# CederGroupHub/smol

Measured on AMD Instinct MI355X. Metric: attempted MC flips/s (node) + ns/flip/replica, 4096-site FCC canonical, higher is better.
Workload: dtype f64

## Files before the change

### smol_amd/codeobj.py

```python

import hashlib
import os
import shutil
import struct
import subprocess

_MAGIC = b"__CLANG_OFFLOAD_BUNDLE__"
_CACHE = {}


def _code_objects(blob):
    pos = blob.find(_MAGIC)
    while pos >= 0:
        (n,) = struct.unpack_from("<Q", blob, pos + len(_MAGIC))
        q = pos + len(_MAGIC) + 8
        for _ in range(n):
            off, size, tlen = struct.unpack_from("<QQQ", blob, q)
            triple = blob[q + 24:q + 24 + tlen].decode()
            q += 24 + tlen
            if triple.startswith("hip") and "amdgcn" in triple and size:
                yield blob[pos + off:pos + off + size]
        pos = blob.find(_MAGIC, pos + len(_MAGIC))


def _elf_symbols(elf):
    if elf[:4] != b"\x7fELF" or elf[4] != 2:
        return [], None
    shoff, = struct.unpack_from("<Q", elf, 0x28)
    shentsize, shnum, _ = struct.unpack_from("<HHH", elf, 0x3A)
    sec = [struct.unpack_from("<IIQQQQIIQQ", elf, shoff + i * shentsize) for i in range(shnum)]
    syms = []
    for s in sec:
        if s[1] != 2:
            continue
        stroff = sec[s[6]][4]
        for k in range(s[5] // 24):
            nm, info, _, shndx, value, size = struct.unpack_from("<IBBHQQ", elf, s[4] + 24 * k)
            end = elf.index(b"\0", stroff + nm)
            syms.append((elf[stroff + nm:end].decode(), info & 0xF, shndx, value, size))

    def read(shndx, value, size):
        s = sec[shndx]
        if s[1] == 8:
            return b""
        o = s[4] + (value - s[3])
        return elf[o:o + size]

    return syms, read


def _demangle(names):
    exe = shutil.which("c++filt") or shutil.which("llvm-cxxfilt") or "/opt/rocm/lib/llvm/bin/llvm-cxxfilt"
    if not (exe and os.path.exists(exe)):
        return list(names)
    out = subprocess.run([exe], input="\n".join(names), capture_output=True, text=True, check=True).stdout
    dem = out.split("\n")[:len(names)]
    return dem if len(dem) == len(names) else list(names)


def _merge_copies(copies):
    return {n: (next(iter(c)) if len(c) == 1 else hashlib.sha256("".join(sorted(c)).encode()).hexdigest())
            for n, c in copies.items()}


def kernel_digests(path=None):
    if path is None:
        from . import engine
        path = os.environ.get("SMOLMC_LIB") or engine.LIB_PATH
    st = os.stat(path)
    key = (os.path.abspath(path), st.st_mtime_ns, st.st_size)
    if key in _CACHE:
        return _CACHE[key]
    with open(path, "rb") as fh:
        blob = fh.read()
    copies = {}
    for elf in _code_objects(blob):
        syms, read = _elf_symbols(elf)
        if read is None:
            continue
        kd = {n[:-3]: (sh, v, sz) for n, t, sh, v, sz in syms if n.endswith(".kd") and 0 < sh < 0xFF00}
        for n, t, sh, v, sz in syms:
            if t != 2 or n not in kd or not (0 < sh < 0xFF00):
                continue
            h = hashlib.sha256()
            h.update(read(sh, v, sz))
            h.update(read(*kd[n]))
            copies.setdefault(n, set()).add(h.hexdigest())
    raw = _merge_copies(copies)
    names = sorted(raw)
    out = {d: raw[m] for m, d in zip(names, _demangle(names))}
    _CACHE[key] = out
    return out


def _norm(name):
    return name.replace(" ", "")


def find_kernel(fragment, path=None):
    f = _norm(fragment)
    hits = [(n, d) for n, d in kernel_digests(path).items() if f in _norm(n)]
    return hits[0] if len(hits) == 1 else None


def isa_stale(entry, path=None):
    if not entry:
        return False
    if entry.get("isa_sha256") and entry.get("kernel_symbol"):
        hit = find_kernel(entry["kernel_symbol"], path)
        return hit is None or hit[1] != entry["isa_sha256"]
    from . import engine
    return entry.get("csrc_sha256") != engine.source_digest()


if __name__ == "__main__":
    import sys

    for name, dig in sorted(kernel_digests(sys.argv[1] if len(sys.argv) > 1 else None).items()):
        print(dig[:16], name[:160])
```

### smol_amd/csrc/mc_lean.h

```cpp
#pragma once
#include "smolmc_common.h"

template <int CTRL> __device__ __forceinline__ double dpp_xor_add(double v) {
    const int lo = __builtin_amdgcn_update_dpp(__double2loint(v), __double2loint(v), CTRL, 0xf, 0xf, true);
    const int hi = __builtin_amdgcn_update_dpp(__double2hiint(v), __double2hiint(v), CTRL, 0xf, 0xf, true);
    return v + __hiloint2double(hi, lo);
}
__device__ __forceinline__ double wave_sum_all(double v) {
    v = dpp_xor_add<0xB1>(v);
    v = dpp_xor_add<0x4E>(v);
    v = dpp_xor_add<0x141>(v);
    v = dpp_xor_add<0x140>(v);
    {
        const unsigned lo = (unsigned)__double2loint(v), hi = (unsigned)__double2hiint(v);
        const auto a = __builtin_amdgcn_permlane16_swap(lo, lo, false, false);
        const auto b = __builtin_amdgcn_permlane16_swap(hi, hi, false, false);
        v = __hiloint2double((int)b[0], (int)a[0]) + __hiloint2double((int)b[1], (int)a[1]);
    }
    {
        const unsigned lo = (unsigned)__double2loint(v), hi = (unsigned)__double2hiint(v);
        const auto a = __builtin_amdgcn_permlane32_swap(lo, lo, false, false);
        const auto b = __builtin_amdgcn_permlane32_swap(hi, hi, false, false);
        v = __hiloint2double((int)b[0], (int)a[0]) + __hiloint2double((int)b[1], (int)a[1]);
    }
    return v;
}

template <int CTRL> __device__ __forceinline__ float dpp_add_f32(float v) {
    const int t = __builtin_amdgcn_update_dpp(0, __float_as_int(v), CTRL, 0xf, 0xf, true);
    return v + __int_as_float(t);
}
__device__ __forceinline__ float wave_sum_f32_uniform(float v) {
    v = dpp_add_f32<0xB1>(v);
    v = dpp_add_f32<0x4E>(v);
    v = dpp_add_f32<0x141>(v);
    v = dpp_add_f32<0x140>(v);
    float total;
    asm volatile("s_nop 1\n\t"
                 "v_add_f32_dpp %1, %1, %1 row_bcast:15 row_mask:0xa bank_mask:0xf\n\t"
                 "s_nop 1\n\t"
                 "v_add_f32_dpp %1, %1, %1 row_bcast:31 row_mask:0xc bank_mask:0xf\n\t"
                 "s_nop 1\n\t"
                 "v_readlane_b32 %0, %1, 63\n\t"
                 "s_nop 1"
                 : "=s"(total), "+v"(v));
    return total;
}

typedef double smolmc_v4d __attribute__((ext_vector_type(4)));
__device__ __forceinline__ double wave_sum_mfma(double v) {
    const smolmc_v4d z = {0.0, 0.0, 0.0, 0.0};
    const smolmc_v4d d = __builtin_amdgcn_mfma_f64_16x16x4f64(v, 1.0, z, 0, 0, 0);
    const double t = (d[0] + d[1]) + (d[2] + d[3]);
    const smolmc_v4d d2 = __builtin_amdgcn_mfma_f64_16x16x4f64(t, 1.0, z, 0, 0, 0);
    return d2[0];
}
#ifdef SMOLMC_MFMA_REDUCE
#define LEAN_WAVE_SUM wave_sum_mfma
#else
#define LEAN_WAVE_SUM wave_sum_all
#endif

__device__ __forceinline__ double lean_ewald_partial(const LeanParams &P, const uint8_t *occ, int lane,
                                                     int s, int swa, int swm, int swb) {
    const double *g = P.ew_G + (size_t)s * P.ew_nact;
    const int W = P.ew_W, na = P.ew_nact;
    double out = 0;
    for (int j0 = lane; j0 < na; j0 += 64 * 8) {
        int k[8];
        double gk[8], q[8];
#pragma unroll
        for (int u = 0; u < 8; ++u) {
            const int jj = min(j0 + 64 * u, na - 1);
            k[u] = P.ew_act[jj];
            gk[u] = g[jj];
        }
#pragma unroll
        for (int u = 0; u < 8; ++u)
            q[u] = P.ew_qs[(size_t)k[u] * W + (int)occ[lean_swz(k[u], swa, swm, swb)]];
#pragma unroll
        for (int u = 0; u < 8; ++u)
            out = fma((j0 + 64 * u < na && k[u] != s) ? q[u] : 0.0, gk[u], out);
    }
    return out;
}

template <int FOOT = 2, bool PRE = false>
__device__ __forceinline__ void field_apply(const LeanParams &P, double *phi, int lane, int s, double dq,
                                            const uint32_t (&e0)[27], const bool have_e0) {
    const int js = s - P.sbase;
    const double keep = phi[js];
    const LeanParamsKernarg Q = rare_params();
    const unsigned char *gx = (const unsigned char *)Q->ew_gx;
    if (gx != nullptr) {
        const uint32_t *E8 = Q->ew_E8;
        const uint32_t s8[1] = {Q->ew_S8[js]};
        const double d[1] = {dq};
        if (PRE && have_e0) field_sweep_gx_pre27(phi, E8, gx, lane, P.ew_nact, s8, d, e0);
        else field_sweep_gx_multi<1, FOOT>(phi, E8, gx, lane, P.ew_nact, s8, d);
    } else {
        const double *g = P.ew_G + (size_t)s * P.ew_nact;
        field_sweep<false>(phi, g, g, lane, P.ew_nact, dq, 0.0);
    }
    phi[js] = keep;
}

template <int FOOT = 2>
__device__ __forceinline__ void field_apply(const LeanParams &P, double *phi, int lane, int s, double dq) {
    const uint32_t none[27] = {};
    field_apply<FOOT, false>(P, phi, lane, s, dq, none, false);
}

template <int FOOT = 1, bool FEW = false>
__device__ __forceinline__ void field_apply_flips(double *phi, int lane, int nfl, int vsite, double vdq) {
    const LeanParamsKernarg Q = rare_params();

    const unsigned char *gx = (const unsigned char *)Q->ew_gx;
    auto site_of = [&](int f) { return (int)rdlane((uint32_t)vsite, f); };
    auto dq_of = [&](int f) {
        return __hiloint2double((int)rdlane((uint32_t)__double2hiint(vdq), f), (int)rdlane((uint32_t)__double2loint(vdq), f));
    };
    const int sb = Q->sbase, na = Q->ew_nact;
    if (gx == nullptr) {
        const double *G = Q->ew_G;
        for (int f = 0; f < nfl; ++f) {
            const double dqf = dq_of(f);
            if (dqf == 0.0) continue;
            const double *g = G + (size_t)site_of(f) * na;
            field_sweep<false>(phi, g, g, lane, na, dqf, 0.0);
        }
        return;
    }
    const uint32_t *E8 = Q->ew_E8, *S8 = Q->ew_S8;
    for (int f0 = 0; f0 < nfl; f0 += 4) {
        const int n = min(4, nfl - f0);
        uint32_t s8[4];
        double dq[4];
#pragma unroll
        for (int k = 0; k < 4; ++k) {
            const int f = k < n ? f0 + k : f0;
            s8[k] = S8[site_of(f) - sb];
            dq[k] = k < n ? dq_of(f) : 0.0;
        }
        if (FEW && n <= 3) {
            const uint32_t a[3] = {s8[0], s8[1], s8[2]};
            const double d[3] = {dq[0], dq[1], dq[2]};
            field_sweep_gx_multi<3, FOOT>(phi, E8, gx, lane, na, a, d);
        } else if (n == 1) {
            const uint32_t a[1] = {s8[0]};
            const double d[1] = {dq[0]};
            field_sweep_gx_multi<1, FOOT>(phi, E8, gx, lane, na, a, d);
        } else if (n == 2) {
            const uint32_t a[2] = {s8[0], s8[1]};
            const double d[2] = {dq[0], dq[1]};
            field_sweep_gx_multi<2, FOOT>(phi, E8, gx, lane, na, a, d);
        } else if (n == 3) {
            const uint32_t a[3] = {s8[0], s8[1], s8[2]};
            const double d[3] = {dq[0], dq[1], dq[2]};
            field_sweep_gx_multi<3, FOOT>(phi, E8, gx, lane, na, a, d);
        } else {
            field_sweep_gx_multi<4, FOOT>(phi, E8, gx, lane, na, s8, dq);
        }
    }
}

template <int FOOT = 1>
__device__ __forceinline__ void field_apply2(const LeanParams &P, double *phi, int lane, int s1, double dq1,
                                             int s2, double dq2) {
    const int j1 = s1 - P.sbase, j2 = s2 - P.sbase;
    const LeanParamsKernarg Q = rare_params();
    const unsigned char *gx = (const unsigned char *)Q->ew_gx;
    if (gx != nullptr) {
        const uint32_t *E8 = Q->ew_E8, *S8 = Q->ew_S8;
        const uint32_t s8[2] = {S8[j1], S8[j2]};
        const double d[2] = {dq1, dq2};
        field_sweep_gx_multi<2, FOOT>(phi, E8, gx, lane, P.ew_nact, s8, d);
        return;
    }
    const double *g1 = P.ew_G + (size_t)s1 * P.ew_nact, *g2 = P.ew_G + (size_t)s2 * P.ew_nact;
    const double keep1 = phi[j1], keep2 = phi[j2];
    const double c12 = g2[j1], c21 = g1[j2];
    field_sweep<true>(phi, g1, g2, lane, P.ew_nact, dq1, dq2);
    if (j1 != j2) {
        phi[j1] = fma(dq2, c12, keep1);
        phi[j2] = fma(dq1, c21, keep2);
    } else {
        phi[j1] = keep1;
    }
}

__device__ __forceinline__ uint32_t bounded(uint32_t a, uint32_t lim) {
#ifdef SMOLMC_BOUNDS
    if (a >= lim) __builtin_trap();
#else
    (void)lim;
#endif
    return a;
}

template <int NW> struct RowWords { uint32_t w[NW]; };
template <int NW>
__device__ __forceinline__ RowWords<NW> load_row(__amdgpu_buffer_rsrc_t rs, uint32_t voff, uint32_t soff) {
    RowWords<NW> r;
    if constexpr (NW == 2) {
        const auto v = __builtin_amdgcn_raw_buffer_load_b64(rs, voff, soff, 0);
        r.w[0] = v[0]; r.w[1] = v[1];
    } else if constexpr (NW == 3) {
        const auto v = __builtin_amdgcn_raw_buffer_load_b96(rs, voff, soff, 0);
        r.w[0] = v[0]; r.w[1] = v[1]; r.w[2] = v[2];
    } else if constexpr (NW == 4) {
        const auto v = __builtin_amdgcn_raw_buffer_load_b128(rs, voff, soff, 0);
        r.w[0] = v[0]; r.w[1] = v[1]; r.w[2] = v[2]; r.w[3] = v[3];
    } else if constexpr (NW == 6) {
        const auto v = __builtin_amdgcn_raw_buffer_load_b128(rs, voff, soff, 0);
        const auto u = __builtin_amdgcn_raw_buffer_load_b64(rs, voff + 16u, soff, 0);
        r.w[0] = v[0]; r.w[1] = v[1]; r.w[2] = v[2]; r.w[3] = v[3]; r.w[4] = u[0]; r.w[5] = u[1];
    } else {
        static_assert(NW % 4 == 0, "row width");
#pragma unroll
        for (int b = 0; b < NW / 4; ++b) {
            const auto v = __builtin_amdgcn_raw_buffer_load_b128(rs, voff + 16u * b, soff, 0);
            r.w[4 * b] = v[0]; r.w[4 * b + 1] = v[1]; r.w[4 * b + 2] = v[2]; r.w[4 * b + 3] = v[3];
        }
    }
    return r;
}
template <int NW> __device__ __forceinline__ uint32_t row_entry(const RowWords<NW> &r, int q) {
    return (r.w[q >> 1] >> (16 * (q & 1))) & 0xffffu;
}
template <bool WIDE, int NW> __device__ __forceinline__ uint32_t row_addr(const RowWords<NW> &r, int q) {
    if constexpr (WIDE) return r.w[q];
    else return row_entry<NW>(r, q);
}

__device__ __noinline__ double wl_flatness_check(const double *wl_S, long long *wl_Hh, int L, double flat,
                                                 double div, double wl_m, int lane) {
    long cnt = 0;
    double sum = 0;
    for (int i = lane; i < L; i += 64)
        if (wl_S[i] > 0) { cnt++; sum += (double)wl_Hh[i]; }
    const double tcnt = wave_sum_all((double)cnt), tsum = wave_sum_all(sum);
    if (tcnt >= 2.0) {
        const double thr = flat * (tsum / tcnt);
        int bad = 0;
        for (int i = lane; i < L; i += 64)
            if (wl_S[i] > 0 && !((double)wl_Hh[i] > thr)) bad = 1;
        if (__ballot(bad) == 0ull) {
            for (int i = lane; i < L; i += 64) wl_Hh[i] = 0;
            wl_m = wl_m / div;
        }
    }
    return wl_m;
}

__device__ __noinline__ double wl_multi_flatness_check(const double *S, uint32_t *cnt, double *occb, long long *hist_g,
                                                       long long *occ_g, int L, double flat, double div, double wl_m, int lane) {
    long n = 0;
    double sum = 0;
    for (int i = lane; i < L; i += 64)
        if (S[i] > 0) { n++; sum += (double)(hist_g[i] + (long long)cnt[i]); }
    const double tn = wave_sum_all((double)n), tsum = wave_sum_all(sum);
    if (tn >= 2.0) {
        const double thr = flat * (tsum / tn);
        int bad = 0;
        for (int i = lane; i < L; i += 64)
            if (S[i] > 0 && !((double)(hist_g[i] + (long long)cnt[i]) > thr)) bad = 1;
        if (__ballot(bad) == 0ull) {
            for (int i = lane; i < L; i += 64) {
                hist_g[i] = 0;
                occ_g[i] += (long long)cnt[i];
                if (occb) occb[i] += (double)cnt[i];
                cnt[i] = 0u;
            }
            wl_m = wl_m / div;
        }
    }
    return wl_m;
}

typedef __attribute__((address_space(3))) uint8_t lds_u8_t;
typedef __attribute__((address_space(3))) double lds_f64_t;
#if defined(__HIP_DEVICE_COMPILE__)
#define SMOLMC_LDS_U8(a) (*(lds_u8_t *)(a))
#define SMOLMC_LDS_F64(a) (*(const lds_f64_t *)(a))
#define SMOLMC_LDS_F32(a) (*(const __attribute__((address_space(3))) float *)(a))
#else
#define SMOLMC_LDS_F32(a) (*(const float *)(uintptr_t)(a))
#define SMOLMC_LDS_U8(a) (*(uint8_t *)(uintptr_t)(a))
#define SMOLMC_LDS_F64(a) (*(const double *)(uintptr_t)(a))
#endif
template <bool ABS> __device__ __forceinline__ uint8_t occ_ld(const uint8_t *occ, uint32_t a) {
    if constexpr (ABS) return SMOLMC_LDS_U8(a);
    else return occ[a];
}
__device__ __forceinline__ uint32_t opaque_u32(uint32_t v) {
    asm volatile("" : "+s"(v));
    return v;
}
template <bool ABS> __device__ __forceinline__ void occ_st(uint8_t *occ, uint32_t a, uint8_t v) {
    if constexpr (ABS) SMOLMC_LDS_U8(a) = v;
    else occ[a] = v;
}

template <int NSLOT, int MM, int STEP, bool HAS_MU, int EWM, bool WL, bool BIAS = false, bool SOLO = false,
          int KF = 0, int OCC = 0, bool REPLAY = false>
__global__ void __attribute__((amdgpu_waves_per_eu(OCC ? OCC : 1, OCC ? OCC : 8)))
__launch_bounds__(256) mc_lean_kernel(const LeanParams P) {
    static_assert(KF == 0 || (!WL && !BIAS && !SOLO), "correlation-function tables: plain Metropolis layouts only");
    static_assert(!REPLAY || (!WL && OCC == 0), "replay: Metropolis variants (Wang-Landau: mc_wl_kernel)");
    constexpr int NACC = KF ? KF : 1;
    constexpr bool HAS_EW = EWM != 0, ew_field = EWM == 2;
    extern __shared__ __attribute__((aligned(16))) unsigned char smem[];
    if ((uint32_t)(uintptr_t)smem != 0u) __builtin_trap();
    const int lane = threadIdx.x & 63;
    const int wave = SOLO ? 0 : threadIdx.x >> 6;
    const int nwaves = SOLO ? 1 : blockDim.x >> 6;
    const int r = uni(blockIdx.x * nwaves + wave);
    const size_t per_wave = (size_t)P.Nlds + 64 * 8 + (WL ? (size_t)P.wl.L * 24 : 0) +
                            ((HAS_EW && ew_field) ? 64 + (size_t)P.ew_nact * 8 : 0);
    double *s_dt = SOLO ? (double *)(smem + ((per_wave + 15) & ~(size_t)15)) : (double *)smem;
    const uint32_t dt_off = SOLO ? (uint32_t)((per_wave + 15) & ~(size_t)15) : 0u;
    double *s_mu = s_dt + P.dt_len;
    double *s_q = s_mu + 8, *s_dg = s_mu + 16;
    unsigned char *wbase = SOLO ? smem : (unsigned char *)(s_mu + 24) + (size_t)wave * per_wave;
    uint8_t *occ = wbase;
    double *s_feat = (double *)(wbase + P.Nlds);
    double *wl_S = s_feat + 64;
    long long *wl_Hh = (long long *)(wl_S + (WL ? P.wl.L : 0));
    long long *wl_Oc = wl_Hh + (WL ? P.wl.L : 0);
    double *phi = (double *)(wbase + P.Nlds + 64 * 8 + 64);
    const int swa = P.swz_a, swm = P.swz_m, swb = P.swz_b;
    for (int i = threadIdx.x; i < P.dt_len; i += blockDim.x) s_dt[i] = P.dt[i];
#ifdef SMOLMC_EXP_F32TAB
    constexpr bool F32TAB = SOLO && STEP == SMOLMC_STEP_SWAP && !HAS_EW && !WL && !BIAS && KF == 0 && !REPLAY;
    const uint32_t sh_off = dt_off + (uint32_t)(P.dt_len + 24) * 8u;
    if (F32TAB) {
        float *s_dt32 = (float *)(smem + sh_off);
        for (int i = threadIdx.x; i < P.dt_len; i += blockDim.x) s_dt32[i] = (float)P.dt[i];
    }
#else
    constexpr bool F32TAB = false;
#endif
    if (HAS_MU && threadIdx.x < 8) s_mu[threadIdx.x] = threadIdx.x < P.ncodes ? P.mu_row[threadIdx.x] : 0.0;
    if (HAS_EW && ew_field && threadIdx.x < 8) {
        s_q[threadIdx.x] = P.ew_qrow[threadIdx.x];
        s_dg[threadIdx.x] = P.ew_dgrow[threadIdx.x];
    }
    const bool live = r < P.R;
    if (live) {
        const uint32_t *src = (const uint32_t *)(P.occ + (size_t)r * P.Npad);
        for (int i = lane; i < P.Npad / 4; i += 64)
            *(uint32_t *)(occ + lean_swz(4 * i, swa, swm, swb)) = src[i];
        s_feat[lane] = (WL && lane < P.F) ? P.features[(size_t)r * P.F + lane] : 0.0;
        if (HAS_EW && ew_field)
            for (int j = lane; j < P.ew_nact; j += 64) phi[j] = P.ew_phi[(size_t)r * P.ew_nact + j];
        if (WL)
            for (int i = lane; i < P.wl.L; i += 64) {
                wl_S[i] = P.wl.entropy[(size_t)r * P.wl.L + i];
                wl_Hh[i] = P.wl.hist[(size_t)r * P.wl.L + i];
                wl_Oc[i] = P.wl.occur[(size_t)r * P.wl.L + i];
            }
    }
    __syncthreads();
    if (!live) return;

#ifdef SMOLMC_NO_EWALD_E8REG
    constexpr bool EPRE = false;
#else
    constexpr bool EPRE = HAS_EW && STEP == SMOLMC_STEP_FLIP && !REPLAY;
#endif
    uint32_t ereg[27] = {};
    bool epre_on = false;
    if (EPRE) {
        const LeanParamsKernarg Q = rare_params();
        const uint32_t *E8 = Q->ew_E8;
        epre_on = ew_field && Q->ew_gx != nullptr && (Q->ew_nact >> 6) >= 27;
        if (epre_on) {
#pragma unroll
            for (int u = 0; u < 27; ++u) ereg[u] = E8[64 * u + lane];
        }
    }

    uint32_t doff8[NSLOT], st8[NSLOT][MM], sfeat[NSLOT];
    double wgt[NSLOT], acc[NSLOT], sfs[NSLOT];
    double accK[NSLOT][NACC];
    uint32_t kslot[NSLOT];
#pragma unroll
    for (int it = 0; it < NSLOT; ++it) {
        const LeanSlot sl = P.slots[it * 64 + lane];
        doff8[it] = sl.doff8 + dt_off;
        sfeat[it] = sl.feat;
        sfs[it] = sl.live ? sl.fs : 0.0;
        kslot[it] = sl.live;
#pragma unroll
        for (int m = 0; m < MM; ++m) st8[it][m] = sl.stride8[m];
        wgt[it] = sl.w;
        acc[it] = 0.0;
#pragma unroll
        for (int k = 0; k < NACC; ++k) accK[it][k] = 0.0;
    }
    const int wl_stride = WL ? P.F : 64;
    const int wl_k = WL ? max(1, min(8, 63 / max(wl_stride, 1))) : 1;
    uint32_t sfeat_wl[NSLOT];
#pragma unroll
    for (int it = 0; it < NSLOT; ++it) sfeat_wl[it] = sfeat[it] + (uint32_t)((lane % wl_k) * wl_stride);
    int wl_rd[8];
#pragma unroll
    for (int k = 0; k < 8; ++k) wl_rd[k] = (WL && k < wl_k && lane < wl_stride) ? lane + k * wl_stride : 63;
    auto wl_cur_feat = [&]() -> double {
        const int f = lane < wl_stride ? lane : 0;
        double t[8];
#pragma unroll
        for (int k = 0; k < 8; ++k) t[k] = k < wl_k ? s_feat[f + (k < wl_k ? k : 0) * wl_stride] : 0.0;
        return ((t[0] + t[1]) + (t[2] + t[3])) + ((t[4] + t[5]) + (t[6] + t[7]));
    };
    auto reduce_features = [&](double *dst) {
#pragma unroll
        for (int it = 0; it < NSLOT; ++it) {
            if (KF == 0) {
                __hip_atomic_fetch_add(&dst[sfeat[it]], sfs[it] * acc[it], __ATOMIC_RELAXED,
                                       __HIP_MEMORY_SCOPE_WAVEFRONT);
            } else {
#pragma unroll
                for (int k = 0; k < NACC; ++k) {
                    const bool on = (uint32_t)k < kslot[it];
                    __hip_atomic_fetch_add(&dst[sfeat[it] + (on ? k : 0)], on ? sfs[it] * accK[it][k] : 0.0,
                                           __ATOMIC_RELAXED, __HIP_MEMORY_SCOPE_WAVEFRONT);
                }
            }
        }
    };
#ifdef SMOLMC_EXP_CLOCK
    const long long ck0 = clock64(), wk0 = wall_clock64();
#endif
    double H = P.enthalpy[r];
    const double nbeta = WL ? 0.0 : -P.beta[r];
    double wl_m = WL ? P.wl.m[r] : 0.0;
    double wl_bq = WL ? floordiv_exact(H - P.wl.vmin, P.wl.bin) : 0.0;
    const double wl_inv_bin = WL ? 1.0 / P.wl.bin : 0.0;
    long long wl_counter = WL ? P.wl.counter[r] : 0;
    long long wl_rem_check = WL ? (P.wl.check ? wl_counter % P.wl.check : 1) : 0;
    unsigned long long step = P.nsteps[r];
    uint32_t nacc_add = 0;
    const uint32_t key0 = (uint32_t)P.seeds[r], key1 = (uint32_t)(P.seeds[r] >> 32);
    const uint32_t nact = (uint32_t)P.nact, nt8 = P.nt8, snt8 = P.snt8;
    const int sbase = P.sbase;
    double acc_mu = 0.0, acc_ew = 0.0;
    const int btype = BIAS ? P.bias_type : 0;
    const int brows = (btype && btype != SMOLMC_BIAS_FUGACITY) ? P.bias_rows : 0;
    double bias_acc = 0.0, chg[SMOLMC_MAX_BIAS_ROWS];
#pragma unroll
    for (int k = 0; k < SMOLMC_MAX_BIAS_ROWS; ++k) chg[k] = k < brows ? P.charge[(size_t)r * SMOLMC_MAX_BIAS_ROWS + k] : 0.0;
    constexpr bool FAST = !WL && !HAS_EW;
    float thr_lo = 0.0f, thr_hi = 0.0f;
    const double inv_nbeta = FAST ? 1.0 / nbeta : 0.0;
    uint32_t nacc_before = 0;
    int nsite = 0, naddr = 0;
    double *featp = P.features + (size_t)r * P.F;
    const double base_feat = lane < P.F ? featp[lane] : 0.0;
    uint32_t smp_countdown = P.smp.every ? (uint32_t)P.smp.every : 0xffffffffu;
    long long smp_index = 0;
    uint32_t W0 = 0;
    int cand[4] = {0, 0, 0, 0}, canda[4] = {0, 0, 0, 0};
    double vGc = 0.0;
    double logu = 0.0;
    unsigned long long batch64_base = ~0ull;
    unsigned long long batch_base = ~0ull;
    constexpr int ROW = NSLOT * MM;
    constexpr int NW = SOLO ? ROW : ROW / 2;
    constexpr uint32_t ENT = SOLO ? 4u : 2u;
    constexpr uint32_t SITE_BYTES = 64u * ROW * ENT;
    const __amdgpu_buffer_rsrc_t idx_rs = __builtin_amdgcn_make_buffer_rsrc(
        SOLO ? (void *)P.idx32 : (void *)P.idx, 0, 0x7fffffff, 0x00020000);
    const uint32_t lane_voff = (uint32_t)lane * (ROW * ENT);

    int s1, a1;
    RowWords<NW> row1;
    uint32_t ridx = 0;
    double lu_rp = 0.0;
    int rp_bad = 0;
    auto rp_site = [&](const uint32_t i) -> int {
        const int v = uni(P.rp_steps[((size_t)r * (uint32_t)P.steps + i) * 4]);
        return v >= 0 ? v : sbase;
    };
    {
        if (REPLAY) {
            s1 = rp_site(0u);
        } else {
            const unsigned long long sp = step - 1ull;
            const uint32_t w = (uint32_t)uni((int)philox4x32_10((uint32_t)sp, (uint32_t)(sp >> 32), 0u, 0u,
                                                                key0, key1).w[1]);
            s1 = sbase + (int)__umulhi(w, nact);
        }
        a1 = lean_swz(s1, swa, swm, swb);
        row1 = load_row<NW>(idx_rs, lane_voff, (uint32_t)s1 * SITE_BYTES);
    }

    double *wl_pend = WL ? P.wl.meanf + (size_t)r * P.wl.L * P.F : nullptr;
    double wl_pc[8] = {0.0, 0.0, 0.0, 0.0, 0.0, 0.0, 0.0, 0.0};
    auto wl_pend_sum = [&]() -> double {
        return ((wl_pc[0] + wl_pc[1]) + (wl_pc[2] + wl_pc[3])) + ((wl_pc[4] + wl_pc[5]) + (wl_pc[6] + wl_pc[7]));
    };
#ifdef SMOLMC_EXP_PHASES
    long long lph[5] = {0, 0, 0, 0, 0};
    long long lph_t = clock64();
#endif
    uint32_t steps_left = (uint32_t)P.steps;
    while (steps_left != 0u) {
        const unsigned long long base = step & ~15ull;
        if (!REPLAY && base != batch_base) {
            batch_base = base;
            const unsigned long long st = base + (unsigned)(lane >> 2);
            const philox_out o = philox4x32_10((uint32_t)st, (uint32_t)(st >> 32), (uint32_t)(lane & 3),
                                               0u, key0, key1);
            W0 = o.w[0];
            nsite = sbase + (int)__umulhi(o.w[1], nact);
            naddr = lean_swz(nsite, swa, swm, swb);
            if ((step & ~63ull) != batch64_base) {
                batch64_base = step & ~63ull;
                const unsigned long long s64 = batch64_base + (unsigned)lane;
                const philox_out a = philox4x32_10((uint32_t)s64, (uint32_t)(s64 >> 32), 0u, 0u, key0, key1);
                logu = log(philox_u53(a.w[2], a.w[3]));
                if (FAST) {
                    const double thr = logu * inv_nbeta;
                    const double eps = (F32TAB ? 2.0 : 1.0) * P.fast_eps + 1e-6 * fabs(thr);
                    thr_lo = P.fast_eps > 0.0 ? (float)(thr - eps) : -INFINITY;
                    thr_hi = P.fast_eps > 0.0 ? (float)(thr + eps) : INFINITY;
                }
            }
            if (STEP == SMOLMC_STEP_SWAP) {
                cand[0] = sbase + (int)__umulhi(o.w[0], nact);
                cand[1] = sbase + (int)__umulhi(o.w[1], nact);
                cand[2] = sbase + (int)__umulhi(o.w[2], nact);
                cand[3] = sbase + (int)__umulhi(o.w[3], nact);
#pragma unroll
                for (int j = 0; j < 4; ++j) canda[j] = lean_swz(cand[j], swa, swm, swb);
                if (HAS_EW && ew_field) {
                    const int prev = __shfl(nsite, (lane & ~3) - 4);
                    const int site_l = lane < 4 ? s1 : prev;
                    vGc = P.ew_G[(size_t)cand[0] * P.ew_nact + (site_l - sbase)];
                }
            }
        }
        uint32_t chunk = 16u - (uint32_t)(step & 15ull);
        chunk = min(chunk, steps_left);
        chunk = min(chunk, smp_countdown);
        steps_left -= chunk;
        smp_countdown -= chunk;
        const unsigned long long chunk_end = step + chunk;
        int l4 = (int)(step & 15ull) * 4;
        int l64 = (int)(step & 63ull);
        do {
#ifndef SMOLMC_NO_SETPRIO
        __builtin_amdgcn_s_setprio(1);
#endif
#ifdef SMOLMC_EXP_PHASES
        { const long long tn = clock64(); lph[0] += tn - lph_t; lph_t = tn; }
#endif
        int s1n, a1n;
        int rq1 = 0, rq2 = -1, rq3 = 0;
        bool rp_empty = false;
        if (REPLAY) {
            const int *rec = P.rp_steps + ((size_t)r * (uint32_t)P.steps + ridx) * 4;
            const int q0 = uni(rec[0]);
            rq1 = uni(rec[1]); rq2 = uni(rec[2]); rq3 = uni(rec[3]);
            rp_empty = q0 < 0;
            double u = uni_d(P.rp_u[(size_t)r * (uint32_t)P.steps + ridx]);
            if (u != u) u = 0.0;
            lu_rp = log(u);
            s1n = ridx + 1u < (uint32_t)P.steps ? rp_site(ridx + 1u) : s1;
            a1n = lean_swz(s1n, swa, swm, swb);
            if (FAST) {
                const double thr = lu_rp * inv_nbeta, eps = P.fast_eps + 1e-6 * fabs(thr);
                thr_lo = P.fast_eps > 0.0 ? (float)(thr - eps) : -INFINITY;
                thr_hi = P.fast_eps > 0.0 ? (float)(thr + eps) : INFINITY;
            }
        } else {
            s1n = (int)rdlane((uint32_t)nsite, l4);
            a1n = (int)rdlane((uint32_t)naddr, l4);
        }
        uint32_t va1 = (uint32_t)a1;
        asm volatile("" : "+v"(va1));
        const int o1 = uni((int)occ_ld<SOLO>(occ, va1));
        int nfl, s2, a2, n1, n2 = 0, o2 = 0;
        if (STEP != SMOLMC_STEP_SWAP) { s2 = s1; a2 = a1; }
        int fb = -1;
        if (REPLAY) {
            if (STEP == SMOLMC_STEP_FLIP) {
                nfl = rp_empty ? 0 : 1;
                n1 = rp_empty ? o1 : rq1;
                rp_bad |= (rq2 >= 0) ? 1 : 0;
            } else if (!rp_empty && rq2 >= 0) {
                nfl = 2;
                s2 = rq2;
                a2 = lean_swz(s2, swa, swm, swb);
                o2 = uni((int)occ_ld<SOLO>(occ, (uint32_t)a2));
                n2 = rq3;
                n1 = rq1;
                rp_bad |= (n2 != o1 || n1 != o2) ? 1 : 0;
                n2 = o1; n1 = o2;
            } else {
                nfl = 0; s2 = s1; a2 = a1; o2 = o1; n2 = o1; n1 = o1;
                rp_bad |= (!rp_empty || rq2 >= 0) ? 1 : 0;
            }
        } else if (STEP == SMOLMC_STEP_FLIP) {
            const uint32_t kk = __umulhi(rdlane(W0, l4 + 1), (uint32_t)(P.ncodes - 1));
            n1 = (int)kk + ((int)kk >= o1 ? 1 : 0);
            nfl = 1;
        } else {
            nfl = 2;
            n2 = o1;
#define SMOLMC_CAND_MASK(J)                                                                        \
    const int v##J = (int)occ_ld<SOLO>(occ, (uint32_t)canda[J]);                                   \
    const unsigned long long m##J = __ballot(v##J != o1) & (0xEull << l4);
#define SMOLMC_CAND_TAKE(J)                                                                        \
    {                                                                                              \
        const int b = __ffsll((long long)m##J) - 1;                                                \
        s2 = (int)rdlane((uint32_t)cand[J], b);                                                    \
        a2 = (int)rdlane((uint32_t)canda[J], b);                                                   \
        o2 = (int)rdlane((uint32_t)v##J, b);                                                       \
        if (J == 0) fb = b;                                                                        \
    }
            SMOLMC_CAND_MASK(0)
            if (m0) SMOLMC_CAND_TAKE(0)
            else {
                SMOLMC_CAND_MASK(1)
                if (m1) SMOLMC_CAND_TAKE(1)
                else {
                    SMOLMC_CAND_MASK(2)
                    if (m2) SMOLMC_CAND_TAKE(2)
                    else {
                        SMOLMC_CAND_MASK(3)
                        if (m3) SMOLMC_CAND_TAKE(3)
                        else {
                            bool hit = false;
                            const unsigned long long cur = chunk_end - chunk;
                            for (uint32_t q = 0;; ++q) {
                                const philox_out o = philox4x32_10((uint32_t)cur, (uint32_t)(cur >> 32),
                                                                   4u + 64u * q + (uint32_t)lane, 0u, key0, key1);
                                int selsite = -1, selv = 0;
#pragma unroll
                                for (int j = 3; j >= 0; --j) {
                                    const int cs = sbase + (int)__umulhi(o.w[j], nact);
                                    const int v = (int)occ[lean_swz(cs, swa, swm, swb)];
                                    if (v != o1) { selsite = cs; selv = v; }
                                }
                                const unsigned long long m = __ballot(selsite >= 0);
                                if (m) {
                                    const int b = __ffsll((long long)m) - 1;
                                    s2 = (int)rdlane((uint32_t)selsite, b);
                                    a2 = lean_swz(s2, swa, swm, swb);
                                    o2 = (int)rdlane((uint32_t)selv, b);
                                    hit = true;
                                    break;
                                }
                                if ((q & 63u) == 0) {
                                    int any = 0;
                                    for (uint32_t a = lane; a < nact; a += 64)
                                        any |= ((int)occ[lean_swz(sbase + (int)a, swa, swm, swb)] != o1);
                                    if (__ballot(any) == 0ull) break;
                                }
                            }
                            if (!hit) { nfl = 0; s2 = s1; a2 = a1; o2 = o1; }
                        }
                    }
                }
            }
#undef SMOLMC_CAND_MASK
#undef SMOLMC_CAND_TAKE
            n1 = o2;
        }

#ifndef SMOLMC_NO_SETPRIO
        __builtin_amdgcn_s_setprio(2);
#endif
        RowWords<NW> row2 = row1;
        if (STEP == SMOLMC_STEP_SWAP) {
#ifdef SMOLMC_EXP_ROW2
            row2 = load_row<NW>(idx_rs, lane_voff, (uint32_t)s1n * SITE_BYTES);
#else
            row2 = load_row<NW>(idx_rs, lane_voff, (uint32_t)s2 * SITE_BYTES);
#endif
        }
        if (WL) {
            unsafeAtomicAdd(wl_pend + lane, wl_pend_sum());
        }

#ifdef SMOLMC_EXP_PHASES
        { const long long tn = clock64(); lph[1] += tn - lph_t; lph_t = tn; }
#endif
#ifdef SMOLMC_NO_SWAP_DIFF
        constexpr bool DIFF = false;
#else
        constexpr bool DIFF = STEP == SMOLMC_STEP_SWAP;
#endif
        double e = 0.0, d1[NSLOT], d2[NSLOT];
#ifdef SMOLMC_EXP_F32TAB
        float t1f[NSLOT], ef32 = 0.0f;
#endif
        uint32_t dp[NSLOT];
        uint32_t ad1[NSLOT], ad2[NSLOT];
        {
            const uint32_t pair1 = (uint32_t)o1 * snt8 + (uint32_t)n1 * nt8;
#pragma unroll
            for (int it = 0; it < NSLOT; ++it) {
                uint32_t a = doff8[it];
                if (DIFF) a = dp[it] = doff8[it] + pair1;
#pragma unroll
                for (int m = 0; m < MM; ++m) a += __umul24(st8[it][m], (uint32_t)occ_ld<SOLO>(occ, bounded(row_addr<SOLO, NW>(row1, it * MM + m), (uint32_t)P.Nlds)));
                if (DIFF && F32TAB) {
#ifdef SMOLMC_EXP_F32TAB
                    ad1[it] = a;
                    t1f[it] = SMOLMC_LDS_F32(sh_off + ((a - dt_off) >> 1));
#endif
                } else if (DIFF) {
                    d1[it] = SMOLMC_LDS_F64(a);
                    if (KF) ad1[it] = a;
                } else {
                    d1[it] = SMOLMC_LDS_F64(a + pair1);
                    if (KF) ad1[it] = a + pair1;
                    e = fma(wgt[it], d1[it], e);
                }
            }
        }
        row1 = load_row<NW>(idx_rs, lane_voff, (uint32_t)s1n * SITE_BYTES);
        double ew_part = 0.0, ew_uni = 0.0;
        double dq1 = 0.0, dq2 = 0.0;
        if (HAS_EW) {
            if (ew_field) {
                dq1 = s_q[n1] - s_q[o1];
                ew_uni = 2.0 * dq1 * phi[s1 - sbase] + (s_dg[n1] - s_dg[o1]);
            } else {
                const int W = P.ew_W;
                dq1 = P.ew_qs[(size_t)s1 * W + n1] - P.ew_qs[(size_t)s1 * W + o1];
                ew_part = 2.0 * dq1 * lean_ewald_partial(P, occ, lane, s1, swa, swm, swb);
                ew_uni = 2.0 * dq1 * P.ew_frozen[s1] +
                         (P.ew_dg[(size_t)s1 * W + n1] - P.ew_dg[(size_t)s1 * W + o1]);
            }
        }
        if (STEP == SMOLMC_STEP_SWAP) {
#ifndef SMOLMC_EXP_NOTENT
            occ_st<SOLO>(occ, va1, (uint8_t)n1);
#endif
            const uint32_t pair2 = (uint32_t)o2 * snt8 + (uint32_t)n2 * nt8;
#pragma unroll
            for (int it = 0; it < NSLOT; ++it) {
                uint32_t a = DIFF ? dp[it] : doff8[it];
#pragma unroll
                for (int m = 0; m < MM; ++m) a += __umul24(st8[it][m], (uint32_t)occ_ld<SOLO>(occ, bounded(row_addr<SOLO, NW>(row2, it * MM + m), (uint32_t)P.Nlds)));
                if (DIFF && F32TAB) {
#ifdef SMOLMC_EXP_F32TAB
                    ad2[it] = a;
                    ef32 = fmaf((float)wgt[it], t1f[it] - SMOLMC_LDS_F32(sh_off + ((a - dt_off) >> 1)), ef32);
#endif
                } else if (DIFF) {
                    d1[it] -= SMOLMC_LDS_F64(a);
                    if (KF) ad2[it] = a;
                    e = fma(wgt[it], d1[it], e);
                } else {
                    d2[it] = SMOLMC_LDS_F64(a + pair2);
                    if (KF) ad2[it] = a + pair2;
                    e = fma(wgt[it], d2[it], e);
                }
            }
            if (HAS_EW) {
                if (ew_field) {
                    dq2 = s_q[n2] - s_q[o2];
                    const double cross =
                        fb >= 0 ? __hiloint2double((int)rdlane((uint32_t)__double2hiint(vGc), fb),
                                                   (int)rdlane((uint32_t)__double2loint(vGc), fb))
                                : P.ew_G[(size_t)s2 * P.ew_nact + (s1 - sbase)];
                    ew_uni += 2.0 * dq2 * (phi[s2 - sbase] + dq1 * cross) + (s_dg[n2] - s_dg[o2]);
                } else {
                    const int W = P.ew_W;
                    dq2 = P.ew_qs[(size_t)s2 * W + n2] - P.ew_qs[(size_t)s2 * W + o2];
                    ew_part += 2.0 * dq2 * lean_ewald_partial(P, occ, lane, s2, swa, swm, swb);
                    ew_uni += 2.0 * dq2 * P.ew_frozen[s2] +
                              (P.ew_dg[(size_t)s2 * W + n2] - P.ew_dg[(size_t)s2 * W + o2]);
                }
            }
        }
#ifdef SMOLMC_EXP_PHASES
        { const long long tn = clock64(); lph[2] += tn - lph_t; lph_t = tn; }
#endif
        double dMu = 0.0;
        if (HAS_MU && nfl >= 1) {
            dMu = s_mu[n1] - s_mu[o1];
            if (nfl == 2) dMu += s_mu[n2] - s_mu[o2];
        }
        double dH = 0.0, dEw = 0.0;
        double wl_nbq = 0.0;
        double dB = 0.0, dQ[SMOLMC_MAX_BIAS_ROWS] = {0.0, 0.0, 0.0, 0.0};
        if (btype && nfl >= 1) {
            if (btype == SMOLMC_BIAS_FUGACITY) {
                dB = P.bias_pair[o1 * 8 + n1];
                if (nfl == 2) dB += P.bias_pair[o2 * 8 + n2];
            } else {
                double sq_new = 0.0, sq_old = 0.0;
#pragma unroll
                for (int k = 0; k < SMOLMC_MAX_BIAS_ROWS; ++k)
                    if (k < brows) {
                        const double *bp = P.bias_pair + k * P.bias_row_stride;
                        double x = bp[o1 * 8 + n1];
                        if (nfl == 2) x += bp[o2 * 8 + n2];
                        dQ[k] = x;
                        const double cn = chg[k] + x;
                        sq_old += chg[k] * chg[k];
                        sq_new += cn * cn;
                    }
                dB = -P.bias_pen * sq_new - (-P.bias_pen * sq_old);
            }
        }
#ifdef SMOLMC_EXP_F32TAB
        bool have_d1 = false;
#endif
        auto exact_decision = [&]() -> bool {
#ifdef SMOLMC_EXP_F32TAB
            if (F32TAB) {
#pragma unroll
                for (int it = 0; it < NSLOT; ++it) {
                    d1[it] = SMOLMC_LDS_F64(ad1[it]) - SMOLMC_LDS_F64(ad2[it]);
                    e = fma(wgt[it], d1[it], e);
                }
                have_d1 = true;
            }
#endif
            dH = LEAN_WAVE_SUM(e);
            if (HAS_EW) {
                dEw = (ew_field ? 0.0 : LEAN_WAVE_SUM(ew_part)) + ew_uni;
                dH += P.ew_coef * dEw;
            }
            if (HAS_MU) dH -= dMu;
            const double lu = REPLAY ? lu_rp
                                     : __hiloint2double((int)rdlane((uint32_t)__double2hiint(logu), l64),
                                                        (int)rdlane((uint32_t)__double2loint(logu), l64));
            if (!WL) {
                const double exponent = nbeta * dH + 0.0 + dB;
                return __ballot((exponent >= 0.0) || (exponent > lu)) != 0ull;
            } else {
                const double new_h = H + dH;
                if (new_h < P.wl.vmin || new_h >= P.wl.vmax) {
                    return false;
                } else {
                    const int b = (int)wl_bq;
                    wl_nbq = floordiv_exact_inv(new_h - P.wl.vmin, P.wl.bin, wl_inv_bin);
                    const int nb = (int)wl_nbq;
                    const double exponent = wl_S[b] - wl_S[nb] + 0.0;
                    return __ballot((exponent >= 0.0) || (exponent > lu)) != 0ull;
                }
            }
        };
#ifdef SMOLMC_NO_SELACC
        constexpr bool SELACC = false;
#else
        constexpr bool SELACC = DIFF && FAST && !BIAS && !F32TAB;
#endif
        uint32_t sel_hi = 0u;
        auto on_accept = [&]() {
#ifdef SMOLMC_EXP_F32TAB
            if (F32TAB && !have_d1) {
#pragma unroll
                for (int it = 0; it < NSLOT; ++it) d1[it] = SMOLMC_LDS_F64(ad1[it]) - SMOLMC_LDS_F64(ad2[it]);
            }
#endif
            if (KF) {
                const unsigned char *kb = (const unsigned char *)P.dtk;
#pragma unroll
                for (int it = 0; it < NSLOT; ++it) {
                    const uint32_t g1 = doff8[it] * (uint32_t)(SMOLMC_LEAN_MAX_KF - 1) + ad1[it];
                    const uint32_t g2 = doff8[it] * (uint32_t)(SMOLMC_LEAN_MAX_KF - 1) + ad2[it];
#pragma unroll
                    for (int k = 0; k < NACC; ++k) {
                        const bool on = (uint32_t)k < kslot[it];
                        const uint32_t off = (uint32_t)k * P.ktab8;
                        double v = on ? *(const double *)(kb + (g1 + off)) : 0.0;
                        if (STEP == SMOLMC_STEP_SWAP) {
                            const double v2 = on ? *(const double *)(kb + (g2 + off)) : 0.0;
                            v = DIFF ? v - v2 : v + v2;
                        }
                        accK[it][k] += v;
                    }
                }
            }
            if (SELACC) {
                sel_hi = 0x3ff00000u;
            } else if (!WL) {
#pragma unroll
                for (int it = 0; it < NSLOT; ++it) acc[it] += d1[it];
                if (STEP == SMOLMC_STEP_SWAP && !DIFF) {
#pragma unroll
                    for (int it = 0; it < NSLOT; ++it) acc[it] += d2[it];
                }
            } else {
#pragma unroll
                for (int it = 0; it < NSLOT; ++it) {
                    const double dd = (STEP == SMOLMC_STEP_SWAP && !DIFF) ? d1[it] + d2[it] : d1[it];
                    __hip_atomic_fetch_add(&s_feat[sfeat_wl[it]], sfs[it] * dd, __ATOMIC_RELAXED,
                                           __HIP_MEMORY_SCOPE_WAVEFRONT);
                }
            }
            if (STEP == SMOLMC_STEP_FLIP) occ_st<SOLO>(occ, va1, (uint8_t)n1);
#ifdef SMOLMC_EXP_NOTENT
            if (STEP == SMOLMC_STEP_SWAP) occ_st<SOLO>(occ, (uint32_t)a1, (uint8_t)n1);
#endif
            if (STEP == SMOLMC_STEP_SWAP) occ_st<SOLO>(occ, (uint32_t)a2, (uint8_t)n2);
            if (HAS_EW && ew_field) {
                if (STEP == SMOLMC_STEP_SWAP) {
                    if (dq1 != 0.0 || dq2 != 0.0) field_apply2(P, phi, lane, s1, dq1, s2, dq2);
                } else if (dq1 != 0.0) {
#ifndef SMOLMC_EXP_NOFIELD
                    field_apply<2, EPRE>(P, phi, lane, s1, dq1, ereg, epre_on);
#endif
                }
            }
            acc_mu += dMu;
            acc_ew += dEw;
            bias_acc += dB;
#pragma unroll
            for (int k = 0; k < SMOLMC_MAX_BIAS_ROWS; ++k) chg[k] += dQ[k];
            if (!FAST) H += dH;
            if (!SELACC) nacc_add++;
        };
        auto on_reject = [&]() {
            if (STEP == SMOLMC_STEP_SWAP) {
#ifndef SMOLMC_EXP_NOTENT
            occ_st<SOLO>(occ, va1, (uint8_t)o1);
#endif
            }
        };
        nacc_before = nacc_add;
        bool accepted = false;
#ifndef SMOLMC_NO_SETPRIO
        __builtin_amdgcn_s_setprio(3);
#endif
        if (FAST && !BIAS) {
#ifdef SMOLMC_EXP_F32TAB
            const float ef = F32TAB ? ((HAS_MU && lane == 0) ? ef32 - (float)dMu : ef32) : (float)((HAS_MU && lane == 0) ? e - dMu : e);
#else
            const float ef = (float)((HAS_MU && lane == 0) ? e - dMu : e);
#endif
            const float S = wave_sum_f32_uniform(ef);
// ... 1456 lines not shown
```

### smol_amd/csrc/philox.h

```cpp
#pragma once
#include <stdint.h>

#if defined(__HIPCC__)
#define SMOLMC_HD __host__ __device__ __forceinline__
#else
#define SMOLMC_HD inline
#endif

struct philox_out {
    uint32_t w[4];
};

SMOLMC_HD void philox_round(uint32_t &c0, uint32_t &c1, uint32_t &c2, uint32_t &c3, uint32_t k0,
                            uint32_t k1) {
    uint64_t p0 = (uint64_t)0xD2511F53u * c0, p1 = (uint64_t)0xCD9E8D57u * c2;
    uint32_t hi0 = (uint32_t)(p0 >> 32), lo0 = (uint32_t)p0;
    uint32_t hi1 = (uint32_t)(p1 >> 32), lo1 = (uint32_t)p1;
    uint32_t n0 = hi1 ^ c1 ^ k0, n2 = hi0 ^ c3 ^ k1;
    c0 = n0;
    c1 = lo1;
    c2 = n2;
    c3 = lo0;
}

SMOLMC_HD philox_out philox4x32_10(uint32_t c0, uint32_t c1, uint32_t c2, uint32_t c3, uint32_t k0,
                                   uint32_t k1) {
#pragma unroll
    for (int r = 0; r < 10; ++r) {
        philox_round(c0, c1, c2, c3, k0, k1);
        k0 += 0x9E3779B9u;
        k1 += 0xBB67AE85u;
    }
    philox_out o;
    o.w[0] = c0;
    o.w[1] = c1;
    o.w[2] = c2;
    o.w[3] = c3;
    return o;
}

SMOLMC_HD double philox_u53(uint32_t a, uint32_t b) {
    return (double)(((uint64_t)(a >> 5) << 26) | (uint64_t)(b >> 6)) * (1.0 / 9007199254740992.0);
}
```

Measured before the change: 17.81 billion.

## Reuse Philox draws across batches, fuse XORs with bitop3, raise min waves

```diff
diff --git a/smol_amd/codeobj.py b/smol_amd/codeobj.py
--- a/smol_amd/codeobj.py
+++ b/smol_amd/codeobj.py
@@ -113,6 +113,47 @@
     return entry.get("csrc_sha256") != engine.source_digest()
 
 
+def kernel_resources(fragment, path=None):
+    import collections
+    import tempfile
+
+    name = find_kernel(fragment, path)
+    if name is None:
+        return None
+    if path is None:
+        from . import engine
+        path = os.environ.get("SMOLMC_LIB") or engine.LIB_PATH
+    with open(path, "rb") as fh:
+        blob = fh.read()
+    for elf in _code_objects(blob):
+        syms, read = _elf_symbols(elf)
+        if read is None:
+            continue
+        funcs = [(n, sh, v, sz) for n, t, sh, v, sz in syms if t == 2 and 0 < sh < 0xFF00]
+        demangled = _demangle([n for n, *_ in funcs])
+        hit = [f for f, d in zip(funcs, demangled) if d == name[0]]
+        kd = {n[:-3]: (sh, v, sz) for n, t, sh, v, sz in syms if n.endswith(".kd") and 0 < sh < 0xFF00}
+        if not hit or hit[0][0] not in kd:
+            continue
+        desc = read(*kd[hit[0][0]])
+        scratch, = struct.unpack_from("<I", desc, 4)
+        rsrc1, = struct.unpack_from("<I", desc, 48)
+        objdump = shutil.which("llvm-objdump") or "/opt/rocm/lib/llvm/bin/llvm-objdump"
+        with tempfile.NamedTemporaryFile(suffix=".co") as tmp:
+            tmp.write(elf)
+            tmp.flush()
+            out = subprocess.run([objdump, "-d", "--no-show-raw-insn", "--mcpu=gfx950",
+                                  "--disassemble-symbols=" + hit[0][0], tmp.name],
+                                 capture_output=True, text=True, check=True).stdout
+        ops = collections.Counter()
+        for line in out.splitlines():
+            t = line.strip().split()
+            if t and (t[0].startswith(("v_", "s_", "ds_", "buffer_", "global_"))):
+                ops[t[0]] += 1
+        return {"name": name[0], "vgprs": 8 * ((rsrc1 & 0x3F) + 1), "scratch_bytes": scratch, "mnemonics": ops}
+    return None
+
+
 if __name__ == "__main__":
     import sys
 
diff --git a/smol_amd/csrc/mc_lean.h b/smol_amd/csrc/mc_lean.h
--- a/smol_amd/csrc/mc_lean.h
+++ b/smol_amd/csrc/mc_lean.h
@@ -302,9 +302,12 @@
     else occ[a] = v;
 }
 
+template <int NSLOT, int MM, int EWM, bool WL, bool BIAS, int KF, int OCC, bool REPLAY>
+constexpr bool LEAN_RNG_ONCE() { return NSLOT * MM <= 4 && EWM == 0 && !WL && !BIAS && KF == 0 && OCC == 0 && !REPLAY; }
 template <int NSLOT, int MM, int STEP, bool HAS_MU, int EWM, bool WL, bool BIAS = false, bool SOLO = false,
           int KF = 0, int OCC = 0, bool REPLAY = false>
-__global__ void __attribute__((amdgpu_waves_per_eu(OCC ? OCC : 1, OCC ? OCC : 8)))
+__global__ void __attribute__((amdgpu_waves_per_eu(
+    OCC ? OCC : (LEAN_RNG_ONCE<NSLOT, MM, EWM, WL, BIAS, KF, OCC, REPLAY>() ? 4 : 1), OCC ? OCC : 8)))
 __launch_bounds__(256) mc_lean_kernel(const LeanParams P) {
     static_assert(KF == 0 || (!WL && !BIAS && !SOLO), "correlation-function tables: plain Metropolis layouts only");
     static_assert(!REPLAY || (!WL && OCC == 0), "replay: Metropolis variants (Wang-Landau: mc_wl_kernel)");
@@ -460,7 +463,16 @@
     const double base_feat = lane < P.F ? featp[lane] : 0.0;
     uint32_t smp_countdown = P.smp.every ? (uint32_t)P.smp.every : 0xffffffffu;
     long long smp_index = 0;
+#ifdef SMOLMC_RNG_TWICE
+    constexpr bool RNG_ONCE = false;
+#else
+    constexpr bool RNG_ONCE = LEAN_RNG_ONCE<NSLOT, MM, EWM, WL, BIAS, KF, OCC, REPLAY>();
+#endif
+    constexpr bool X3 = LEAN_RNG_ONCE<NSLOT, MM, EWM, WL, BIAS, KF, OCC, REPLAY>();
     uint32_t W0 = 0;
+    uint32_t pw1 = 0, pw2 = 0, pw3 = 0;
+    uint32_t pmask = 0u;
+
     int cand[4] = {0, 0, 0, 0}, canda[4] = {0, 0, 0, 0};
     double vGc = 0.0;
     double logu = 0.0;
@@ -488,7 +500,7 @@
             s1 = rp_site(0u);
         } else {
             const unsigned long long sp = step - 1ull;
-            const uint32_t w = (uint32_t)uni((int)philox4x32_10((uint32_t)sp, (uint32_t)(sp >> 32), 0u, 0u,
+            const uint32_t w = (uint32_t)uni((int)philox4x32_10<X3>((uint32_t)sp, (uint32_t)(sp >> 32), 0u, 0u,
                                                                 key0, key1).w[1]);
             s1 = sbase + (int)__umulhi(w, nact);
         }
@@ -510,23 +522,46 @@
         const unsigned long long base = step & ~15ull;
         if (!REPLAY && base != batch_base) {
             batch_base = base;
-            const unsigned long long st = base + (unsigned)(lane >> 2);
-            const philox_out o = philox4x32_10((uint32_t)st, (uint32_t)(st >> 32), (uint32_t)(lane & 3),
+            const unsigned long long st = base + (unsigned)(lane >> 2) + (RNG_ONCE && (lane & 3) == 0 ? 64u : 0u);
+            const philox_out o = philox4x32_10<X3>((uint32_t)st, (uint32_t)(st >> 32), (uint32_t)(lane & 3),
                                                0u, key0, key1);
             W0 = o.w[0];
-            nsite = sbase + (int)__umulhi(o.w[1], nact);
-            naddr = lean_swz(nsite, swa, swm, swb);
+            if (!RNG_ONCE) {
+                nsite = sbase + (int)__umulhi(o.w[1], nact);
+                naddr = lean_swz(nsite, swa, swm, swb);
+            }
             if ((step & ~63ull) != batch64_base) {
                 batch64_base = step & ~63ull;
-                const unsigned long long s64 = batch64_base + (unsigned)lane;
-                const philox_out a = philox4x32_10((uint32_t)s64, (uint32_t)(s64 >> 32), 0u, 0u, key0, key1);
-                logu = log(philox_u53(a.w[2], a.w[3]));
+                uint32_t b1, b2, b3;
+                if (RNG_ONCE && pmask == 0xFu) {
+                    b1 = pw1; b2 = pw2; b3 = pw3;
+                } else {
+                    const unsigned long long s64 = batch64_base + (unsigned)lane;
+                    const philox_out a = philox4x32_10<X3>((uint32_t)s64, (uint32_t)(s64 >> 32), 0u, 0u, key0, key1);
+                    b1 = a.w[1]; b2 = a.w[2]; b3 = a.w[3];
+                }
+                pmask = 0u;
+                logu = log(philox_u53(b2, b3));
                 if (FAST) {
                     const double thr = logu * inv_nbeta;
                     const double eps = (F32TAB ? 2.0 : 1.0) * P.fast_eps + 1e-6 * fabs(thr);
                     thr_lo = P.fast_eps > 0.0 ? (float)(thr - eps) : -INFINITY;
                     thr_hi = P.fast_eps > 0.0 ? (float)(thr + eps) : INFINITY;
                 }
+                if (RNG_ONCE) {
+                    nsite = sbase + (int)__umulhi(b1, nact);
+                    naddr = lean_swz(nsite, swa, swm, swb);
+                }
+            }
+            if (RNG_ONCE) {
+                const int q = (int)(base >> 4) & 3;
+                const int src = (lane & 15) * 4;
+                const uint32_t g1 = __shfl(o.w[1], src), g2 = __shfl(o.w[2], src), g3 = __shfl(o.w[3], src);
+                const bool mine = (lane >> 4) == q;
+                pw1 = mine ? g1 : pw1;
+                pw2 = mine ? g2 : pw2;
+                pw3 = mine ? g3 : pw3;
+                pmask |= 1u << q;
             }
             if (STEP == SMOLMC_STEP_SWAP) {
                 cand[0] = sbase + (int)__umulhi(o.w[0], nact);
@@ -536,7 +571,8 @@
 #pragma unroll
                 for (int j = 0; j < 4; ++j) canda[j] = lean_swz(cand[j], swa, swm, swb);
                 if (HAS_EW && ew_field) {
-                    const int prev = __shfl(nsite, (lane & ~3) - 4);
+                    const int prev = RNG_ONCE ? __shfl(nsite, (int)(base & 63ull) + (lane >> 2) - 1)
+                                              : __shfl(nsite, (lane & ~3) - 4);
                     const int site_l = lane < 4 ? s1 : prev;
                     vGc = P.ew_G[(size_t)cand[0] * P.ew_nact + (site_l - sbase)];
                 }
@@ -576,8 +612,8 @@
                 thr_hi = P.fast_eps > 0.0 ? (float)(thr + eps) : INFINITY;
             }
         } else {
-            s1n = (int)rdlane((uint32_t)nsite, l4);
-            a1n = (int)rdlane((uint32_t)naddr, l4);
+            s1n = (int)rdlane((uint32_t)nsite, RNG_ONCE ? l64 : l4);
+            a1n = (int)rdlane((uint32_t)naddr, RNG_ONCE ? l64 : l4);
         }
         uint32_t va1 = (uint32_t)a1;
         asm volatile("" : "+v"(va1));
@@ -636,7 +672,7 @@
                             bool hit = false;
                             const unsigned long long cur = chunk_end - chunk;
                             for (uint32_t q = 0;; ++q) {
-                                const philox_out o = philox4x32_10((uint32_t)cur, (uint32_t)(cur >> 32),
+                                const philox_out o = philox4x32_10<X3>((uint32_t)cur, (uint32_t)(cur >> 32),
                                                                    4u + 64u * q + (uint32_t)lane, 0u, key0, key1);
                                 int selsite = -1, selv = 0;
 #pragma unroll
diff --git a/smol_amd/csrc/philox.h b/smol_amd/csrc/philox.h
--- a/smol_amd/csrc/philox.h
+++ b/smol_amd/csrc/philox.h
@@ -11,23 +11,35 @@
     uint32_t w[4];
 };
 
+template <bool X3 = false>
 SMOLMC_HD void philox_round(uint32_t &c0, uint32_t &c1, uint32_t &c2, uint32_t &c3, uint32_t k0,
                             uint32_t k1) {
     uint64_t p0 = (uint64_t)0xD2511F53u * c0, p1 = (uint64_t)0xCD9E8D57u * c2;
     uint32_t hi0 = (uint32_t)(p0 >> 32), lo0 = (uint32_t)p0;
     uint32_t hi1 = (uint32_t)(p1 >> 32), lo1 = (uint32_t)p1;
-    uint32_t n0 = hi1 ^ c1 ^ k0, n2 = hi0 ^ c3 ^ k1;
+    uint32_t n0, n2;
+#if defined(__HIP_DEVICE_COMPILE__) && defined(__gfx950__) && !defined(SMOLMC_NO_BITOP3)
+    if (X3) {
+        n0 = __builtin_amdgcn_bitop3_b32(hi1, c1, k0, 0x96);
+        n2 = __builtin_amdgcn_bitop3_b32(hi0, c3, k1, 0x96);
+    } else
+#endif
+    {
+        n0 = hi1 ^ c1 ^ k0;
+        n2 = hi0 ^ c3 ^ k1;
+    }
     c0 = n0;
     c1 = lo1;
     c2 = n2;
     c3 = lo0;
 }
 
+template <bool X3 = false>
 SMOLMC_HD philox_out philox4x32_10(uint32_t c0, uint32_t c1, uint32_t c2, uint32_t c3, uint32_t k0,
                                    uint32_t k1) {
 #pragma unroll
     for (int r = 0; r < 10; ++r) {
-        philox_round(c0, c1, c2, c3, k0, k1);
+        philox_round<X3>(c0, c1, c2, c3, k0, k1);
         k0 += 0x9E3779B9u;
         k1 += 0xBB67AE85u;
     }
```

After: 17.84 billion, median of 6. No clear change (+0.2%).
